# simplify23/MRN

Measured on AMD Instinct MI355X. Metric: text-line images/sec (fwd+bwd) at 32x256, TRBA+MRN 6 experts, higher is better.
Workload: dtype f32; 1 GPU; MRN loop B: TRBAx6 frozen experts fwd + DM-Router fwd/bwd + clip + Adam, 32x256x4 crops; per_gpu_batch=256, global_batch=256, parallelism=dp1

## Files before the change

mrn_amd/_lib.py:

```python
import ctypes
import os
import re

import torch

_HERE = os.path.dirname(os.path.abspath(__file__))
LIB_PATH = os.environ.get("MRN_LIB_PATH") or os.path.join(_HERE, "csrc", "libmrn_hip.so")
HEADER_PATH = os.path.join(os.path.dirname(_HERE), "include", "mrn_hip.h")
DECODE_HEADER_PATH = os.path.join(os.path.dirname(_HERE), "include", "mrn_decode.h")
ATTN_BEAM_HEADER_PATH = os.path.join(os.path.dirname(_HERE), "include", "mrn_attn_beam.h")
LEXICON_HEADER_PATH = os.path.join(os.path.dirname(_HERE), "include", "mrn_lexicon.h")
ATTN_LEXICON_HEADER_PATH = os.path.join(os.path.dirname(_HERE), "include", "mrn_attn_lexicon.h")

_CTYPES = {
    "int": ctypes.c_int,
    "int64_t": ctypes.c_int64,
    "float": ctypes.c_float,
    "void*": ctypes.c_void_p,
    "float*": ctypes.c_void_p,
    "const float*": ctypes.c_void_p,
    "const int64_t*": ctypes.c_void_p,
    "int64_t*": ctypes.c_void_p,
    "const int*": ctypes.c_void_p,
    "int*": ctypes.c_void_p,
    "const int32_t*": ctypes.c_void_p,
    "int32_t*": ctypes.c_void_p,
    "const void*": ctypes.c_void_p,
    "const void* const*": ctypes.c_void_p,
    "const char*": ctypes.c_char_p,
}


def parse_header(path=HEADER_PATH):
    text = open(path).read()
    text = re.sub(r"/\*.*?\*/", "", text, flags=re.S)
    text = re.sub(r"//[^\n]*", "", text)
    protos = {}
    for m in re.finditer(r"(?m)^\s*((?:const\s+)?\w+\s*\*?)\s*(mrn_\w+)\s*\(([^;{]*?)\)\s*;", text):
        ret = re.sub(r"\s+", " ", m.group(1)).strip().replace(" *", "*")
        name = m.group(2)
        args = m.group(3).strip()
        argtypes, argnames = [], []
        if args and args != "void":
            for a in args.split(","):
                a = re.sub(r"\s+", " ", a).strip()
                mm = re.match(r"(.*?)(\w+)$", a)
                ty = mm.group(1).strip().replace(" *", "*")
                argtypes.append(ty)
                argnames.append(mm.group(2))
        protos[name] = (ret, argtypes, argnames)
    return protos


class _Lib:
    def __init__(self):
        self._dll = None
        self._protos = None

    def load(self):
        if self._dll is not None:
            return self._dll
        if not os.path.exists(LIB_PATH):
            raise RuntimeError(
                f"{LIB_PATH} is missing: build it with `python -m mrn_amd.build` (there is no CPU fallback)")
        dll = ctypes.CDLL(LIB_PATH)
        self._protos = {**parse_header(), **parse_header(DECODE_HEADER_PATH), **parse_header(ATTN_BEAM_HEADER_PATH),
                        **parse_header(LEXICON_HEADER_PATH), **parse_header(ATTN_LEXICON_HEADER_PATH)}
        for name, (ret, argtypes, _) in self._protos.items():
            fn = getattr(dll, name)
            fn.restype = _CTYPES[ret]
            fn.argtypes = [_CTYPES[t] for t in argtypes]
        self._dll = dll
        return dll

    def call(self, name, *args):
        dll = self.load()
        fn = getattr(dll, name)
        rc = fn(*args)
        if fn.restype is ctypes.c_int and rc != 0:
            msg = dll.mrn_last_error().decode()
            raise RuntimeError(f"{name} failed (code {rc}): {msg}")
        return rc


LIB = _Lib()


def call(name, *args):
    return LIB.call(name, *args)
```

mrn_amd/csrc/group_ops.hip:

```cpp
#include "common.hpp"

namespace {

typedef _Float16 f16v8 __attribute__((ext_vector_type(8)));
typedef _Float16 f16v4 __attribute__((ext_vector_type(4)));

struct F8 {
  f32x4 a, b;
};

__device__ __forceinline__ F8 load8(const float* p) {
  F8 v;
  v.a = *reinterpret_cast<const f32x4*>(p);
  v.b = *reinterpret_cast<const f32x4*>(p + 4);
  return v;
}
__device__ __forceinline__ void store8(float* p, const F8& v) {
  *reinterpret_cast<f32x4*>(p) = v.a;
  *reinterpret_cast<f32x4*>(p + 4) = v.b;
}
__device__ __forceinline__ void store_hl(unsigned char* out, long row, int C, int c8, const F8& v) {
  f16v8 h, l;
#pragma unroll
  for (int e = 0; e < 4; ++e) {
    _Float16 hh, ll;
    split_f16_sat(v.a[e], hh, ll);
    h[e] = hh; l[e] = ll;
    split_f16_sat(v.b[e], hh, ll);
    h[4 + e] = hh; l[4 + e] = ll;
  }
  unsigned char* o = out + (row * (C >> 5) + (c8 >> 2)) * 128 + (c8 & 3) * 16;
  *reinterpret_cast<f16v8*>(o) = h;
  *reinterpret_cast<f16v8*>(o + 64) = l;
// ... 141 lines not shown
    }
    if (res || res_hl) {
      F8 r = res ? load8(res + i * 8) : load_hl(res_hl, row, C, c8);
      if constexpr (AFFINE) {
        const F8 rs = load8(res_scale + (long)g * C + c8 * 8), rt = load8(res_shift + (long)g * C + c8 * 8);
#pragma unroll
        for (int e = 0; e < 4; ++e) {
          r.a[e] = r.a[e] * rs.a[e] + rt.a[e];
          r.b[e] = r.b[e] * rs.b[e] + rt.b[e];
        }
      }
#pragma unroll
      for (int e = 0; e < 4; ++e) {
        v.a[e] += r.a[e];
        v.b[e] += r.b[e];
      }
    }
    if (relu == 1) {
#pragma unroll
      for (int e = 0; e < 4; ++e) {
        v.a[e] = relu_nan(v.a[e]);
        v.b[e] = relu_nan(v.b[e]);
      }
    } else if (relu == 2) {
#pragma unroll
      for (int e = 0; e < 4; ++e) {
        v.a[e] = 0.5f * v.a[e] * (1.f + erff(v.a[e] * 0.70710678118654752440f));
        v.b[e] = 0.5f * v.b[e] * (1.f + erff(v.b[e] * 0.70710678118654752440f));
      }
    }
    if (out) store8(out + i * 8, v);
    if (out_hl) store_hl(out_hl, row, C, c8, v);
  }
}

template <int R, bool AFFINE>
__global__ __launch_bounds__(256) void bn_apply_wino_grouped_kernel(const float* __restrict__ y, const float* __restrict__ res,
                                                                    const unsigned char* __restrict__ res_hl,
                                                                    const float* __restrict__ res_scale,
                                                                    const float* __restrict__ res_shift,
                                                                    const float* __restrict__ scale, const float* __restrict__ shift,
                                                                    float* __restrict__ out, unsigned char* __restrict__ out_hl,
                                                                    unsigned char* __restrict__ out_v, long imgrows_per_group, int W,
                                                                    int Wq, long n8, int C, int relu,
                                                                    const float* __restrict__ prescale, int dense) {
  constexpr int NC = R + 2;
  const float ps = prescale ? prescale[0] : 1.f;
  const int C8 = C >> 3, Cb = C >> 5;
  for (long i = blockIdx.x * 256L + threadIdx.x; i < n8; i += (long)gridDim.x * 256) {
    const int c8 = (int)(i % C8);
    const long t = i / C8;
    const int q = (int)(t % Wq);
    const long irow = t / Wq;
    const int g = (int)(irow / imgrows_per_group);
    F8 sc, sh;
    if (scale) {
      sc = load8(scale + (long)g * C + c8 * 8);
      sh = load8(shift + (long)g * C + c8 * 8);
    }
    F8 rs, rt;
    if constexpr (AFFINE) {
      rs = load8(res_scale + (long)g * C + c8 * 8);
      rt = load8(res_shift + (long)g * C + c8 * 8);
    }
    F8 d[NC];
#pragma unroll
    for (int j = 0; j < NC; ++j) {
      const int x = R * q - 1 + j;
      if ((unsigned)x < (unsigned)W) {
        const long row = irow * W + x;
        F8 v = load8(y + (row * C8 + c8) * 8);
        if (scale) {
#pragma unroll
          for (int e = 0; e < 4; ++e) {
            v.a[e] = v.a[e] * sc.a[e] + sh.a[e];
            v.b[e] = v.b[e] * sc.b[e] + sh.b[e];
          }
        }
        if (res || res_hl) {
          F8 r = res ? load8(res + (row * C8 + c8) * 8) : load_hl(res_hl, row, C, c8);
          if constexpr (AFFINE) {
#pragma unroll
            for (int e = 0; e < 4; ++e) {
              r.a[e] = r.a[e] * rs.a[e] + rt.a[e];
              r.b[e] = r.b[e] * rs.b[e] + rt.b[e];
            }
          }
#pragma unroll
          for (int e = 0; e < 4; ++e) {
            v.a[e] += r.a[e];
            v.b[e] += r.b[e];
          }
        }
        if (relu) {
#pragma unroll
          for (int e = 0; e < 4; ++e) {
            v.a[e] = relu_nan(v.a[e]);
            v.b[e] = relu_nan(v.b[e]);
          }
        }
        if (j >= 1 && j <= R) {
          if (out) store8(out + (row * C8 + c8) * 8, v);
          if (out_hl) store_hl(out_hl, row, C, c8, v);
        }
        d[j] = v;
      } else {
#pragma unroll
        for (int e = 0; e < 4; ++e) d[j].a[e] = d[j].b[e] = 0.f;
      }
    }
    F8 m[NC];
#pragma unroll
    for (int e = 0; e < 8; ++e) {
      auto D = [&](int j) { return e < 4 ? d[j].a[e] : d[j].b[e - 4]; };
      float r_[NC];
      if constexpr (R == 2) {
        r_[0] = D(0) - D(2);
        r_[1] = D(1) + D(2);
        r_[2] = D(2) - D(1);
        r_[3] = D(1) - D(3);
      } else {
        r_[0] = 4.f * D(0) - 5.f * D(2) + D(4);
        r_[1] = -4.f * (D(1) + D(2)) + D(3) + D(4);
        r_[2] = 4.f * (D(1) - D(2)) - D(3) + D(4);
        r_[3] = 2.f * (D(3) - D(1)) - D(2) + D(4);
        r_[4] = 2.f * (D(1) - D(3)) - D(2) + D(4);
        r_[5] = 4.f * D(1) - 5.f * D(3) + D(5);
      }
#pragma unroll
      for (int k = 0; k < NC; ++k) {
        if (e < 4) m[k].a[e] = r_[k] * ps;
        else m[k].b[e - 4] = r_[k] * ps;
      }
    }
#pragma unroll
    for (int k = 0; k < NC; ++k) {
      if (dense) store_d16(out_v, t * NC + k, C, c8, m[k], dense);
      else store_hl(out_v, t * NC + k, C, c8, m[k]);
    }
  }
}

__global__ __launch_bounds__(256) void maxpool_grouped_kernel(const float* __restrict__ x, const float* __restrict__ scale,
                                                              const float* __restrict__ shift, float* __restrict__ out,
                                                              unsigned char* __restrict__ out_hl, int relu, int B, long n8,
                                                              int H, int W, int C, int Ho, int Wo, int kh, int kw, int sh,
                                                              int sw, int ph, int pw) {
  const int C8 = C >> 3;
  for (long i = blockIdx.x * 256L + threadIdx.x; i < n8; i += (long)gridDim.x * 256) {
    const int c8 = (int)(i % C8);
    const long row = i / C8;
    long r = row;
    const int ox = (int)(r % Wo);
    r /= Wo;
    const int oy = (int)(r % Ho);
    const long b = r / Ho;
    const int g = (int)(b / B);
    F8 sc, sf;
    if (scale) {
      sc = load8(scale + (long)g * C + c8 * 8);
      sf = load8(shift + (long)g * C + c8 * 8);
    }
    F8 m;
#pragma unroll
    for (int e = 0; e < 4; ++e) m.a[e] = m.b[e] = -INFINITY;
    for (int ky = 0; ky < kh; ++ky) {
      const int iy = oy * sh - ph + ky;
      if ((unsigned)iy >= (unsigned)H) continue;
      for (int kx = 0; kx < kw; ++kx) {
        const int ix = ox * sw - pw + kx;
        if ((unsigned)ix >= (unsigned)W) continue;
// ... 30 lines not shown
                                                                   unsigned char* __restrict__ out_hl, unsigned char* __restrict__ out_v,
                                                                   int relu, int B, long n8, int H, int W, int C, int Ho, int Wo, int Wq,
                                                                   int kh, int kw, int sh, int sw, int ph, int pw, int dense) {
  constexpr int NC = R + 2;
  const int C8 = C >> 3;
  for (long i = blockIdx.x * 256L + threadIdx.x; i < n8; i += (long)gridDim.x * 256) {
    const int c8 = (int)(i % C8);
    const long t = i / C8;
    const int q = (int)(t % Wq);
    const long prow = t / Wq;
    const int oy = (int)(prow % Ho);
    const long b = prow / Ho;
    const int g = (int)(b / B);
    F8 sc, sf;
    if (scale) {
      sc = load8(scale + (long)g * C + c8 * 8);
      sf = load8(shift + (long)g * C + c8 * 8);
    }
    F8 d[NC];
#pragma unroll
    for (int j = 0; j < NC; ++j) {
      const int ox = R * q - 1 + j;
      if ((unsigned)ox < (unsigned)Wo) {
        F8 m;
#pragma unroll
        for (int e = 0; e < 4; ++e) m.a[e] = m.b[e] = -INFINITY;
        for (int ky = 0; ky < kh; ++ky) {
          const int iy = oy * sh - ph + ky;
          if ((unsigned)iy >= (unsigned)H) continue;
          for (int kx = 0; kx < kw; ++kx) {
            const int ix = ox * sw - pw + kx;
            if ((unsigned)ix >= (unsigned)W) continue;
            F8 v = load8(x + (((b * H + iy) * W + ix) * (long)C8 + c8) * 8);
            if (scale) {
#pragma unroll
              for (int e = 0; e < 4; ++e) {
                v.a[e] = v.a[e] * sc.a[e] + sf.a[e];
                v.b[e] = v.b[e] * sc.b[e] + sf.b[e];
              }
            }
#pragma unroll
            for (int e = 0; e < 4; ++e) {
              m.a[e] = max_nan(m.a[e], v.a[e]);
              m.b[e] = max_nan(m.b[e], v.b[e]);
            }
          }
        }
        if (relu) {
#pragma unroll
          for (int e = 0; e < 4; ++e) {
            m.a[e] = relu_nan(m.a[e]);
            m.b[e] = relu_nan(m.b[e]);
          }
        }
        if (j >= 1 && j <= R) {
          const long row = prow * Wo + ox;
          if (out) store8(out + (row * C8 + c8) * 8, m);
          if (out_hl) store_hl(out_hl, row, C, c8, m);
        }
        d[j] = m;
      } else {
#pragma unroll
        for (int e = 0; e < 4; ++e) d[j].a[e] = d[j].b[e] = 0.f;
      }
    }
    F8 m_[NC];
#pragma unroll
    for (int e = 0; e < 8; ++e) {
      auto D = [&](int j) { return e < 4 ? d[j].a[e] : d[j].b[e - 4]; };
      float r_[NC];
      if constexpr (R == 2) {
        r_[0] = D(0) - D(2);
        r_[1] = D(1) + D(2);
        r_[2] = D(2) - D(1);
        r_[3] = D(1) - D(3);
      } else {
        r_[0] = 4.f * D(0) - 5.f * D(2) + D(4);
        r_[1] = -4.f * (D(1) + D(2)) + D(3) + D(4);
        r_[2] = 4.f * (D(1) - D(2)) - D(3) + D(4);
        r_[3] = 2.f * (D(3) - D(1)) - D(2) + D(4);
        r_[4] = 2.f * (D(1) - D(3)) - D(2) + D(4);
        r_[5] = 4.f * D(1) - 5.f * D(3) + D(5);
      }
#pragma unroll
      for (int k = 0; k < NC; ++k) {
        if (e < 4) m_[k].a[e] = r_[k];
        else m_[k].b[e - 4] = r_[k];
      }
    }
#pragma unroll
    for (int k = 0; k < NC; ++k) {
      if (dense) store_d16(out_v, t * NC + k, C, c8, m_[k], dense);
      else store_hl(out_v, t * NC + k, C, c8, m_[k]);
    }
  }
}

template <int LPR>
__global__ __launch_bounds__(256) void add_layernorm_grouped_kernel(const float* __restrict__ x, const float* __restrict__ branch,
                                                                   const float* __restrict__ drop, long rows_per_drop,
                                                                   const float* __restrict__ gamma, const float* __restrict__ beta,
                                                                   long rows_per_group, float* __restrict__ sum_out,
                                                                   float* __restrict__ y_f32, unsigned char* __restrict__ y_hl,
                                                                   long rows, int C, float eps) {
  constexpr int RPW = 64 / LPR;
  constexpr int NV = 4;
  const int lane = threadIdx.x & 63, sub = lane % LPR;
  const long row = (blockIdx.x * 4L + (threadIdx.x >> 6)) * RPW + lane / LPR;
  if (row >= rows) return;
  const int C4 = C >> 2;
  const float* xr = x + row * C;
  f32x4 v[NV];
  float s = 0.f;
  const float ds = (branch && drop) ? drop[row / rows_per_drop] : 1.f;
#pragma unroll
  for (int i = 0; i < NV; ++i) {
    const int c4 = sub + i * LPR;
    v[i] = f32x4{0.f, 0.f, 0.f, 0.f};
    if (c4 < C4) {
      v[i] = reinterpret_cast<const f32x4*>(xr)[c4];
      if (branch) {
        const f32x4 b = reinterpret_cast<const f32x4*>(branch + row * C)[c4];
#pragma unroll
        for (int j = 0; j < 4; ++j) v[i][j] = fmaf(ds, b[j], v[i][j]);
      }
      if (sum_out) reinterpret_cast<f32x4*>(sum_out + row * C)[c4] = v[i];
// ... 177 lines not shown
                           const float* res_shift, const float* scale, const float* shift, float* out_f32, void* out_hl32, int G,
                           int64_t rows_per_group, int C, int relu, void* stream) {
  MRN_CHECK_ARG(y && (out_f32 || out_hl32) && C % 8 == 0 && (!(out_hl32 || residual_hl32) || C % 32 == 0) &&
                    (!scale == !shift) && !(residual && residual_hl32),
                "mrn_bn_apply_grouped_f32: bad operands (C=%d)", C);
  MRN_CHECK_ARG((!res_scale == !res_shift) && (!res_scale || (residual && !residual_hl32)),
                "mrn_bn_apply_grouped_res_affine_f32: the residual affine needs both vectors and the fp32 residual (C=%d)", C);
  const long n8 = (long)G * rows_per_group * (C / 8);
  if (n8 == 0) return MRN_OK;
  long grid = (n8 + 255) / 256;
  if (grid > 32768) grid = 32768;
  auto kernel = res_scale ? bn_apply_grouped_kernel<true> : bn_apply_grouped_kernel<false>;
  hipLaunchKernelGGL(kernel, dim3((unsigned)grid), dim3(256), 0, (hipStream_t)stream, y, residual,
                     (const unsigned char*)residual_hl32, res_scale, res_shift, scale, shift,
                     out_f32, (unsigned char*)out_hl32, (long)rows_per_group, n8, C, relu);
  MRN_LAUNCH_CHECK("bn_apply_grouped");
  return MRN_OK;
}

MRN_EXPORT int mrn_bn_apply_grouped_f32(const float* y, const float* residual, const void* residual_hl32, const float* scale,
                                        const float* shift, float* out_f32, void* out_hl32, int G, int64_t rows_per_group,
                                        int C, int relu, void* stream) {
  return bn_apply_launch(y, residual, residual_hl32, nullptr, nullptr, scale, shift, out_f32, out_hl32, G, rows_per_group, C, relu, stream);
}

MRN_EXPORT int mrn_bn_apply_grouped_res_affine_f32(const float* y, const float* residual, const void* residual_hl32,
                                                   const float* scale, const float* shift, float* out_f32, void* out_hl32, int G,
                                                   int64_t rows_per_group, int C, int relu, const float* res_scale,
                                                   const float* res_shift, void* stream) {
  return bn_apply_launch(y, residual, residual_hl32, res_scale, res_shift, scale, shift, out_f32, out_hl32, G, rows_per_group, C, relu,
                         stream);
}

static int bn_apply_wino_launch(const float* y, const float* residual, const void* residual_hl32, const float* res_scale,
                                const float* res_shift, const float* scale, const float* shift, float* out_f32, void* out_hl32,
                                void* out_wino, int G, int B, int H, int W, int C, int R, int relu, const float* prescale, int dense,
                                void* stream) {
  MRN_CHECK_ARG(y && out_wino && C % (dense ? 64 : 32) == 0 && (!scale == !shift) && !(residual && residual_hl32) && (R == 2 || R == 4) &&
                    out_f32 != y && (uintptr_t)out_wino % 128 == 0,
                "mrn_bn_apply_wino_grouped_f32: bad operands (C=%d R=%d)", C, R);
  MRN_CHECK_ARG((!res_scale == !res_shift) && (!res_scale || (residual && !residual_hl32)),
                "mrn_bn_apply_wino_grouped_res_affine_f32: the residual affine needs both vectors and the fp32 residual (C=%d)", C);
  const int Wq = (W + R - 1) / R;
  const long n8 = (long)G * B * H * Wq * (C / 8);
  if (n8 == 0) return MRN_OK;
  long grid = (n8 + 255) / 256;
  if (grid > 32768) grid = 32768;
  auto kernel = R == 4 ? (res_scale ? bn_apply_wino_grouped_kernel<4, true> : bn_apply_wino_grouped_kernel<4, false>)
                       : (res_scale ? bn_apply_wino_grouped_kernel<2, true> : bn_apply_wino_grouped_kernel<2, false>);
  hipLaunchKernelGGL(kernel, dim3((unsigned)grid), dim3(256), 0, (hipStream_t)stream, y, residual, (const unsigned char*)residual_hl32,
                     res_scale, res_shift, scale, shift, out_f32, (unsigned char*)out_hl32, (unsigned char*)out_wino, (long)B * H, W, Wq,
                     n8, C, relu, prescale, dense);
  MRN_LAUNCH_CHECK("bn_apply_wino_grouped");
  return MRN_OK;
}

MRN_EXPORT int mrn_bn_apply_wino_grouped_f32(const float* y, const float* residual, const void* residual_hl32, const float* scale,
                                             const float* shift, float* out_f32, void* out_hl32, void* out_wino, int G, int B, int H,
                                             int W, int C, int R, int relu, const float* prescale, void* stream) {
  return bn_apply_wino_launch(y, residual, residual_hl32, nullptr, nullptr, scale, shift, out_f32, out_hl32, out_wino, G, B, H, W, C, R, relu,
                              prescale, 0, stream);
}

MRN_EXPORT int mrn_bn_apply_wino_grouped_res_affine_f32(const float* y, const float* residual, const void* residual_hl32,
                                                        const float* scale, const float* shift, float* out_f32, void* out_hl32,
                                                        void* out_wino, int G, int B, int H, int W, int C, int R, int relu,
                                                        const float* prescale, const float* res_scale, const float* res_shift,
                                                        void* stream) {
  return bn_apply_wino_launch(y, residual, residual_hl32, res_scale, res_shift, scale, shift, out_f32, out_hl32, out_wino, G, B, H, W, C, R,
                              relu, prescale, 0, stream);
}

MRN_EXPORT int mrn_bn_apply_wino_grouped_d16_f32(const float* y, const float* residual, const void* residual_hl32, const float* scale,
                                                 const float* shift, float* out_f32, void* out_hl32, void* out_wino_d16, int G, int B, int H,
                                                 int W, int C, int relu, const float* prescale, int bf16, void* stream) {
  return bn_apply_wino_launch(y, residual, residual_hl32, nullptr, nullptr, scale, shift, out_f32, out_hl32, out_wino_d16, G, B, H, W, C, 4,
                              relu, prescale, bf16 ? 2 : 1, stream);
}

MRN_EXPORT int mrn_bn_apply_wino_grouped_d16_res_affine_f32(const float* y, const float* residual, const void* residual_hl32,
                                                            const float* scale, const float* shift, float* out_f32, void* out_hl32,
                                                            void* out_wino_d16, int G, int B, int H, int W, int C, int relu,
                                                            const float* prescale, int bf16, const float* res_scale,
                                                            const float* res_shift, void* stream) {
  return bn_apply_wino_launch(y, residual, residual_hl32, res_scale, res_shift, scale, shift, out_f32, out_hl32, out_wino_d16, G, B, H, W,
                              C, 4, relu, prescale, bf16 ? 2 : 1, stream);
}

MRN_EXPORT int mrn_maxpool_grouped_f32(const float* x, const float* scale, const float* shift, int relu, float* out_f32,
                                       void* out_hl32, int G, int B, int H, int W, int C, int kh, int kw, int sh, int sw, int ph,
                                       int pw, void* stream) {
  MRN_CHECK_ARG(x && (out_f32 || out_hl32) && C % 8 == 0 && (!out_hl32 || C % 32 == 0) && (!scale == !shift),
                "mrn_maxpool_grouped_f32: bad operands (C=%d)", C);
  const int Ho = (H + 2 * ph - kh) / sh + 1, Wo = (W + 2 * pw - kw) / sw + 1;
  MRN_CHECK_ARG(Ho > 0 && Wo > 0, "mrn_maxpool_grouped_f32: empty output");
  const long n8 = (long)G * B * Ho * Wo * (C / 8);
  if (n8 == 0) return MRN_OK;
  long grid = (n8 + 255) / 256;
  if (grid > 32768) grid = 32768;
  hipLaunchKernelGGL(maxpool_grouped_kernel, dim3((unsigned)grid), dim3(256), 0, (hipStream_t)stream, x, scale, shift, out_f32,
                     (unsigned char*)out_hl32, relu, B, n8, H, W, C, Ho, Wo, kh, kw, sh, sw, ph, pw);
  MRN_LAUNCH_CHECK("maxpool_grouped");
  return MRN_OK;
}

static int maxpool_wino_launch(const float* x, const float* scale, const float* shift, int relu, float* out_f32,
                               void* out_hl32, void* out_wino, int G, int B, int H, int W, int C, int kh, int kw, int sh,
                               int sw, int ph, int pw, int R, int dense, void* stream) {
  MRN_CHECK_ARG(x && out_wino && C % (dense ? 64 : 32) == 0 && (!scale == !shift) && (R == 2 || R == 4) && (uintptr_t)out_wino % 128 == 0,
                "mrn_maxpool_wino_grouped_f32: bad operands (C=%d R=%d)", C, R);
  const int Ho = (H + 2 * ph - kh) / sh + 1, Wo = (W + 2 * pw - kw) / sw + 1;
  MRN_CHECK_ARG(Ho > 0 && Wo > 0, "mrn_maxpool_wino_grouped_f32: empty output");
  const int Wq = (Wo + R - 1) / R;
  const long n8 = (long)G * B * Ho * Wq * (C / 8);
  if (n8 == 0) return MRN_OK;
  long grid = (n8 + 255) / 256;
  if (grid > 32768) grid = 32768;
  if (R == 4)
    hipLaunchKernelGGL(maxpool_wino_grouped_kernel<4>, dim3((unsigned)grid), dim3(256), 0, (hipStream_t)stream, x, scale, shift, out_f32,
                       (unsigned char*)out_hl32, (unsigned char*)out_wino, relu, B, n8, H, W, C, Ho, Wo, Wq, kh, kw, sh, sw, ph, pw, dense);
  else
    hipLaunchKernelGGL(maxpool_wino_grouped_kernel<2>, dim3((unsigned)grid), dim3(256), 0, (hipStream_t)stream, x, scale, shift, out_f32,
                       (unsigned char*)out_hl32, (unsigned char*)out_wino, relu, B, n8, H, W, C, Ho, Wo, Wq, kh, kw, sh, sw, ph, pw, dense);
  MRN_LAUNCH_CHECK("maxpool_wino_grouped");
  return MRN_OK;
}

MRN_EXPORT int mrn_maxpool_wino_grouped_f32(const float* x, const float* scale, const float* shift, int relu, float* out_f32,
                                            void* out_hl32, void* out_wino, int G, int B, int H, int W, int C, int kh, int kw, int sh,
                                            int sw, int ph, int pw, int R, void* stream) {
  return maxpool_wino_launch(x, scale, shift, relu, out_f32, out_hl32, out_wino, G, B, H, W, C, kh, kw, sh, sw, ph, pw, R, 0, stream);
}

MRN_EXPORT int mrn_maxpool_wino_grouped_d16_f32(const float* x, const float* scale, const float* shift, int relu, float* out_f32,
                                                void* out_hl32, void* out_wino_d16, int G, int B, int H, int W, int C, int kh, int kw, int sh,
                                                int sw, int ph, int pw, int bf16, void* stream) {
  return maxpool_wino_launch(x, scale, shift, relu, out_f32, out_hl32, out_wino_d16, G, B, H, W, C, kh, kw, sh, sw, ph, pw, 4, bf16 ? 2 : 1, stream);
}

MRN_EXPORT int mrn_add_layernorm_grouped_f32(const float* x, const float* branch, const float* drop, int64_t rows_per_drop,
                                             const float* gamma, const float* beta, int64_t rows_per_group, float* sum_out,
                                             float* y_f32, void* y_hl32, int64_t rows, int C, float eps, void* stream) {
  MRN_CHECK_ARG(x && (y_f32 || y_hl32 || sum_out) && C % 4 == 0 && C <= 1024 && (!y_hl32 || C % 32 == 0) && (!gamma == !beta) &&
                    rows_per_group >= 1 && (!drop || rows_per_drop >= 1),
                "mrn_add_layernorm_grouped_f32: bad operands (C=%d)", C);
  if (rows == 0) return MRN_OK;
  const hipStream_t st = (hipStream_t)stream;
  unsigned char* hl = (unsigned char*)y_hl32;
#define MRN_ALN_LAUNCH(LPR)                                                                                                   \
  hipLaunchKernelGGL(add_layernorm_grouped_kernel<LPR>, dim3((unsigned)((rows + 4 * (64 / LPR) - 1) / (4 * (64 / LPR)))),     \
                     dim3(256), 0, st, x, branch, drop, (long)rows_per_drop, gamma, beta, (long)rows_per_group, sum_out, y_f32,  \
// ... 9 lines not shown
```

mrn_amd/ops.py:

```python
import os
import sys
import weakref

import torch

from ._lib import call
from .modules.label_length import ctc_label_length_supported, ctc_uses_long_kernel, unsupported_label_length_message
from .modules.task_count import router_uses_wide_kernels, tasks_supported, unsupported_task_count_message

ACT_NONE, ACT_RELU, ACT_GELU = 0, 1, 2


class KernelTimer:

    def __init__(self, only=None):
        self.spans = []
        self.only = only

    def begin(self, site="other"):
        if self.only is not None and site not in self.only:
            return None
        e = torch.cuda.Event(enable_timing=True)
        e.record()
        return e
# ... 560 lines not shown
        else:
            call("mrn_pack_weight_wino_hl32", _p(w), out.data_ptr() + g * per, O, I, R, scale[g].data_ptr(), _stream())
    return out, scale


def bn_apply_wino_grouped(y, scale, shift, R, relu=True, residual=None, residual_hl=None, want_f32=False, want_hl=False, prescale=None,
                          dense=None, residual_affine=None):
    G, B, H, W, C = y.shape
    Wq = (W + R - 1) // R
    dense = wino_dense() if dense is None else dense
    eb = 2 if dense else 4
    out = torch.empty_like(y) if want_f32 else None
    out_hl = torch.empty(y.numel() * 4, device=y.device, dtype=torch.uint8) if want_hl else None
    v = torch.empty(G * B * H * Wq * (R + 2) * C * eb, device=y.device, dtype=torch.uint8)
    t0 = CONV_TIMER.begin("bnw") if CONV_TIMER is not None else None
    if residual_affine is not None:
        rs, rt = _residual_affine(residual_affine, residual, G, C)
        if dense:
            call("mrn_bn_apply_wino_grouped_d16_res_affine_f32", _p(y), _p(residual), _p(residual_hl), _p(scale), _p(shift), _p(out),
                 _p(out_hl), _p(v), G, B, H, W, C, int(bool(relu)), _p(prescale), int(REDUCED_BF16), _p(rs), _p(rt), _stream())
        else:
            call("mrn_bn_apply_wino_grouped_res_affine_f32", _p(y), _p(residual), _p(residual_hl), _p(scale), _p(shift), _p(out),
                 _p(out_hl), _p(v), G, B, H, W, C, R, int(bool(relu)), _p(prescale), _p(rs), _p(rt), _stream())
    elif dense:
        call("mrn_bn_apply_wino_grouped_d16_f32", _p(y), _p(residual), _p(residual_hl), _p(scale), _p(shift), _p(out), _p(out_hl), _p(v),
             G, B, H, W, C, int(bool(relu)), _p(prescale), int(REDUCED_BF16), _stream())
    else:
        call("mrn_bn_apply_wino_grouped_f32", _p(y), _p(residual), _p(residual_hl), _p(scale), _p(shift), _p(out), _p(out_hl), _p(v),
             G, B, H, W, C, R, int(bool(relu)), _p(prescale), _stream())
    if t0 is not None:
        n_io = 1 + int(residual is not None or residual_hl is not None) + int(want_f32) + int(want_hl)
        CONV_TIMER.end(t0, 0.0, "hbm/bn_apply_wino_grouped", 4.0 * y.numel() * n_io + float(eb) * G * B * H * Wq * (R + 2) * C)
    return out, out_hl, v


def wino_pool_supported(H, W, R, Cout):
    return PATCH_CONV and H % 2 == 0 and W % 2 == 0 and bool(call("mrn_conv2d_x3_wino_rows", H, R, Cout))


def conv2d_x3_wino(v_hl, G, shared_input, B, H, W, Cin, u_hl, u_scale, Cout, R, bias=None, act=ACT_NONE, want_stats=False, out=None,
                   x_scale=None, pool=False, gamma_ptrs=None, dense=None):
    dev = v_hl.device
    y = out if out is not None else torch.empty(G, B, H // 2 if pool else H, W // 2 if pool else W, Cout, device=dev, dtype=torch.float32)
    stats = None
    if want_stats:
        stats = torch.empty(call("mrn_conv2d_x3_wino_stats_floats", G, B, H, W, Cout, R), device=dev, dtype=torch.float32)
    Wq = (W + R - 1) // R
    dense = wino_dense() if dense is None else dense
    eb = 2 if dense else 4
    gstride = 0 if shared_input else B * H * Wq * (R + 2) * Cin * eb
    timed = CONV_TIMER is not None
    t0 = CONV_TIMER.begin("wino") if timed else None
    if dense:
        call("mrn_conv2d_x3_wino_d16", _p(v_hl), _p(u_hl), _p(bias), _p(y), _p(stats), _p(u_scale), _p(x_scale), G, gstride, B, H, W, Cin,
             Cout, act, int(bool(pool)), _p(gamma_ptrs), int(REDUCED_BF16), _stream())
    elif pool:
        call("mrn_conv2d_x3_wino_pool_hl32", _p(v_hl), _p(u_hl), _p(_zero_page(dev)), _p(bias), _p(y), _p(stats), _p(u_scale), _p(x_scale), G,
             gstride, B, H, W, Cin, Cout, R, act, _p(gamma_ptrs), _stream())
    else:
        call("mrn_conv2d_x3_wino_hl32", _p(v_hl), _p(u_hl), _p(_zero_page(dev)), _p(bias), _p(y), _p(stats), _p(u_scale), _p(x_scale), G,
             gstride, B, H, W, Cin, Cout, R, act, _stream())
    if WINO_CHECK and not pool and not dense and call("mrn_conv2d_x3_wino_rows", H, R, Cout):
        call("mrn_conv2d_x3_wino_select", 0)
        y2 = torch.empty_like(y)
        st2 = torch.empty(call("mrn_conv2d_x3_wino_stats_floats", G, B, H, W, Cout, R), device=dev, dtype=torch.float32) if want_stats else None
        call("mrn_conv2d_x3_wino_hl32", _p(v_hl), _p(u_hl), _p(_zero_page(dev)), _p(bias), _p(y2), _p(st2), _p(u_scale), _p(x_scale), G, gstride,
# ... 1854 lines not shown
```

Before: 3133 images/s.

## Walk Winograd tiles sequentially per thread to reuse overlapping BN and pool columns

The Winograd input producers (BN-apply and maxpool) now let each thread walk a run of consecutive tiles along a row. The overlapping halo columns carry over in registers instead of being reloaded and recomputed for every tile, and the next tile's loads are prefetched. Pooling windows also keep their overlapping columns between outputs. Split mode is chosen from C and Wq, or from an env var or select call. This cuts redundant global loads and recomputation, but lowers parallelism and raises register pressure.

Result: no change. 3140 images/s (median of 6 runs) (+0.2%).

```diff
diff --git a/include/mrn_wino_producer.h b/include/mrn_wino_producer.h
--- /dev/null
+++ b/include/mrn_wino_producer.h
@@ -0,0 +1,15 @@
+#ifndef MRN_WINO_PRODUCER_H
+#define MRN_WINO_PRODUCER_H
+#include <stdint.h>
+
+#ifdef __cplusplus
+extern "C" {
+#endif
+
+int mrn_wino_producer_select(int mode);
+int mrn_wino_producer_plan(int64_t rows, int Wq, int C, int split, int part, int64_t* plan);
+
+#ifdef __cplusplus
+}
+#endif
+#endif
diff --git a/mrn_amd/_lib.py b/mrn_amd/_lib.py
--- a/mrn_amd/_lib.py
+++ b/mrn_amd/_lib.py
@@ -11,6 +11,7 @@
 ATTN_BEAM_HEADER_PATH = os.path.join(os.path.dirname(_HERE), "include", "mrn_attn_beam.h")
 LEXICON_HEADER_PATH = os.path.join(os.path.dirname(_HERE), "include", "mrn_lexicon.h")
 ATTN_LEXICON_HEADER_PATH = os.path.join(os.path.dirname(_HERE), "include", "mrn_attn_lexicon.h")
+WINO_PRODUCER_HEADER_PATH = os.path.join(os.path.dirname(_HERE), "include", "mrn_wino_producer.h")
 
 _CTYPES = {
     "int": ctypes.c_int,
@@ -65,7 +66,8 @@
                 f"{LIB_PATH} is missing: build it with `python -m mrn_amd.build` (there is no CPU fallback)")
         dll = ctypes.CDLL(LIB_PATH)
         self._protos = {**parse_header(), **parse_header(DECODE_HEADER_PATH), **parse_header(ATTN_BEAM_HEADER_PATH),
-                        **parse_header(LEXICON_HEADER_PATH), **parse_header(ATTN_LEXICON_HEADER_PATH)}
+                        **parse_header(LEXICON_HEADER_PATH), **parse_header(ATTN_LEXICON_HEADER_PATH),
+                        **parse_header(WINO_PRODUCER_HEADER_PATH)}
         for name, (ret, argtypes, _) in self._protos.items():
             fn = getattr(dll, name)
             fn.restype = _CTYPES[ret]
diff --git a/mrn_amd/csrc/group_ops.hip b/mrn_amd/csrc/group_ops.hip
--- a/mrn_amd/csrc/group_ops.hip
+++ b/mrn_amd/csrc/group_ops.hip
@@ -1,4 +1,5 @@
 #include "common.hpp"
+#include <stdlib.h>
 
 namespace {
 
@@ -206,6 +207,151 @@
     if (out) store8(out + i * 8, v);
     if (out_hl) store_hl(out_hl, row, C, c8, v);
   }
+}
+
+
+struct WinoRaw {
+  F8 y, r;
+};
+
+__device__ __forceinline__ WinoRaw bnw_load(const float* __restrict__ y, const float* __restrict__ res,
+                                            const unsigned char* __restrict__ res_hl, long row, int C, int C8, int c8) {
+  WinoRaw w;
+  w.y = load8(y + (row * C8 + c8) * 8);
+  if (res) {
+    w.r = load8(res + (row * C8 + c8) * 8);
+  } else if (res_hl) {
+    const unsigned char* o = res_hl + (row * (C >> 5) + (c8 >> 2)) * 128 + (c8 & 3) * 16;
+    w.r.a = *reinterpret_cast<const f32x4*>(o);
+    w.r.b = *reinterpret_cast<const f32x4*>(o + 64);
+  }
+  return w;
+}
+
+template <bool AFFINE>
+__device__ __forceinline__ F8 bnw_eval(const WinoRaw& w, bool has_scale, bool res_f32, bool res_hl, const F8& sc, const F8& sh,
+                                       const F8& rs, const F8& rt, int relu) {
+  F8 v = w.y;
+  if (has_scale) {
+#pragma unroll
+    for (int e = 0; e < 4; ++e) {
+      v.a[e] = v.a[e] * sc.a[e] + sh.a[e];
+      v.b[e] = v.b[e] * sc.b[e] + sh.b[e];
+    }
+  }
+  if (res_f32 || res_hl) {
+    F8 r;
+    if (res_f32) {
+      r = w.r;
+    } else {
+      const f16v8 h = __builtin_bit_cast(f16v8, w.r.a), l = __builtin_bit_cast(f16v8, w.r.b);
+#pragma unroll
+      for (int e = 0; e < 4; ++e) {
+        r.a[e] = (float)h[e] + (float)l[e];
+        r.b[e] = (float)h[4 + e] + (float)l[4 + e];
+      }
+    }
+    if constexpr (AFFINE) {
+#pragma unroll
+      for (int e = 0; e < 4; ++e) {
+        r.a[e] = r.a[e] * rs.a[e] + rt.a[e];
+        r.b[e] = r.b[e] * rs.b[e] + rt.b[e];
+      }
+    }
+#pragma unroll
+    for (int e = 0; e < 4; ++e) {
+      v.a[e] += r.a[e];
+      v.b[e] += r.b[e];
+    }
+  }
+  if (relu) {
+#pragma unroll
+    for (int e = 0; e < 4; ++e) {
+      v.a[e] = relu_nan(v.a[e]);
+      v.b[e] = relu_nan(v.b[e]);
+    }
+  }
+  return v;
+}
+
+__device__ __forceinline__ F8 zero8() {
+  F8 z;
+#pragma unroll
+  for (int e = 0; e < 4; ++e) z.a[e] = z.b[e] = 0.f;
+  return z;
+}
+
+template <int R>
+__device__ __forceinline__ float wino_bt(int k, float d0, float d1, float d2, float d3, float d4, float d5) {
+  if constexpr (R == 2) {
+    switch (k) {
+      case 0: return d0 - d2;
+      case 1: return d1 + d2;
+      case 2: return d2 - d1;
+      default: return d1 - d3;
+    }
+  } else {
+    switch (k) {
+      case 0: return 4.f * d0 - 5.f * d2 + d4;
+      case 1: return -4.f * (d1 + d2) + d3 + d4;
+      case 2: return 4.f * (d1 - d2) - d3 + d4;
+      case 3: return 2.f * (d3 - d1) - d2 + d4;
+      case 4: return 2.f * (d1 - d3) - d2 + d4;
+      default: return 4.f * d1 - 5.f * d3 + d5;
+    }
+  }
+}
+
+template <int R, bool PRESCALE, bool SEQ>
+__device__ __forceinline__ void wino_bt_store(const F8 (&d)[R + 2], float ps, unsigned char* __restrict__ out_v, long t, int C, int c8,
+                                              int dense) {
+  constexpr int NC = R + 2;
+#pragma unroll
+  for (int k = 0; k < NC; ++k) {
+    F8 m;
+#pragma unroll
+    for (int e = 0; e < 8; ++e) {
+      auto D = [&](int j) { return e < 4 ? d[j < NC ? j : NC - 1].a[e] : d[j < NC ? j : NC - 1].b[e - 4]; };
+      const float r_ = wino_bt<R>(k, D(0), D(1), D(2), D(3), D(4), D(5));
+      const float val = PRESCALE ? r_ * ps : r_;
+      if (e < 4) m.a[e] = val;
+      else m.b[e - 4] = val;
+    }
+    if (dense) store_d16(out_v, t * NC + k, C, c8, m, dense);
+    else store_hl(out_v, t * NC + k, C, c8, m);
+    if (SEQ) __builtin_amdgcn_sched_barrier(0);
+  }
+}
+
+__device__ __forceinline__ F8 pool_affine(F8 v, const F8& sc, const F8& sf) {
+#pragma unroll
+  for (int e = 0; e < 4; ++e) {
+    v.a[e] = v.a[e] * sc.a[e] + sf.a[e];
+    v.b[e] = v.b[e] * sc.b[e] + sf.b[e];
+  }
+  return v;
+}
+__device__ __forceinline__ F8 pool_max(F8 m, const F8& v) {
+#pragma unroll
+  for (int e = 0; e < 4; ++e) {
+    m.a[e] = max_nan(m.a[e], v.a[e]);
+    m.b[e] = max_nan(m.b[e], v.b[e]);
+  }
+  return m;
+}
+__device__ __forceinline__ F8 relu8(F8 m) {
+#pragma unroll
+  for (int e = 0; e < 4; ++e) {
+    m.a[e] = relu_nan(m.a[e]);
+    m.b[e] = relu_nan(m.b[e]);
+  }
+  return m;
+}
+
+__host__ __device__ inline void wino_walk_run(int Wq, int split, int part, int& q0, int& q1) {
+  const int base = Wq / split, rem = Wq % split;
+  q0 = part * base + (part < rem ? part : rem);
+  q1 = q0 + base + (part < rem ? 1 : 0);
 }
 
 template <int R, bool AFFINE>
@@ -243,74 +389,102 @@
       const int x = R * q - 1 + j;
       if ((unsigned)x < (unsigned)W) {
         const long row = irow * W + x;
-        F8 v = load8(y + (row * C8 + c8) * 8);
-        if (scale) {
-#pragma unroll
-          for (int e = 0; e < 4; ++e) {
-            v.a[e] = v.a[e] * sc.a[e] + sh.a[e];
-            v.b[e] = v.b[e] * sc.b[e] + sh.b[e];
-          }
-        }
-        if (res || res_hl) {
-          F8 r = res ? load8(res + (row * C8 + c8) * 8) : load_hl(res_hl, row, C, c8);
-          if constexpr (AFFINE) {
-#pragma unroll
-            for (int e = 0; e < 4; ++e) {
-              r.a[e] = r.a[e] * rs.a[e] + rt.a[e];
-              r.b[e] = r.b[e] * rs.b[e] + rt.b[e];
-            }
-          }
-#pragma unroll
-          for (int e = 0; e < 4; ++e) {
-            v.a[e] += r.a[e];
-            v.b[e] += r.b[e];
-          }
-        }
-        if (relu) {
-#pragma unroll
-          for (int e = 0; e < 4; ++e) {
-            v.a[e] = relu_nan(v.a[e]);
-            v.b[e] = relu_nan(v.b[e]);
-          }
-        }
+        const F8 v = bnw_eval<AFFINE>(bnw_load(y, res, res_hl, row, C, C8, c8), scale != nullptr, res != nullptr, res_hl != nullptr, sc, sh,
+                                      rs, rt, relu);
         if (j >= 1 && j <= R) {
           if (out) store8(out + (row * C8 + c8) * 8, v);
           if (out_hl) store_hl(out_hl, row, C, c8, v);
         }
         d[j] = v;
       } else {
-#pragma unroll
-        for (int e = 0; e < 4; ++e) d[j].a[e] = d[j].b[e] = 0.f;
-      }
-    }
-    F8 m[NC];
-#pragma unroll
-    for (int e = 0; e < 8; ++e) {
-      auto D = [&](int j) { return e < 4 ? d[j].a[e] : d[j].b[e - 4]; };
-      float r_[NC];
-      if constexpr (R == 2) {
-        r_[0] = D(0) - D(2);
-        r_[1] = D(1) + D(2);
-        r_[2] = D(2) - D(1);
-        r_[3] = D(1) - D(3);
-      } else {
-        r_[0] = 4.f * D(0) - 5.f * D(2) + D(4);
-        r_[1] = -4.f * (D(1) + D(2)) + D(3) + D(4);
-        r_[2] = 4.f * (D(1) - D(2)) - D(3) + D(4);
-        r_[3] = 2.f * (D(3) - D(1)) - D(2) + D(4);
-        r_[4] = 2.f * (D(1) - D(3)) - D(2) + D(4);
-        r_[5] = 4.f * D(1) - 5.f * D(3) + D(5);
-      }
-#pragma unroll
-      for (int k = 0; k < NC; ++k) {
-        if (e < 4) m[k].a[e] = r_[k] * ps;
-        else m[k].b[e - 4] = r_[k] * ps;
-      }
-    }
-#pragma unroll
-    for (int k = 0; k < NC; ++k) {
-      if (dense) store_d16(out_v, t * NC + k, C, c8, m[k], dense);
-      else store_hl(out_v, t * NC + k, C, c8, m[k]);
+        d[j] = zero8();
+      }
+    }
+    wino_bt_store<R, true, false>(d, ps, out_v, t, C, c8, dense);
+  }
+}
+
+template <int R, bool AFFINE, int SPLIT, int RES>
+__global__ __launch_bounds__(256) void bn_apply_wino_grouped_kernel(const float* __restrict__ y, const float* __restrict__ res_,
+                                                                    const unsigned char* __restrict__ res_hl_,
+                                                                    const float* __restrict__ res_scale,
+                                                                    const float* __restrict__ res_shift,
+                                                                    const float* __restrict__ scale, const float* __restrict__ shift,
+                                                                    float* __restrict__ out, unsigned char* __restrict__ out_hl,
+                                                                    unsigned char* __restrict__ out_v, long imgrows_per_group, int W,
+                                                                    int Wq, long n8, int C, int relu,
+                                                                    const float* __restrict__ prescale, int dense) {
+  constexpr int NC = R + 2;
+  const float ps = prescale ? prescale[0] : 1.f;
+  const int C8 = C >> 3;
+  const float* __restrict__ res = RES == 1 ? res_ : nullptr;
+  const unsigned char* __restrict__ res_hl = RES == 2 ? res_hl_ : nullptr;
+  const bool has_scale = scale != nullptr, res_f32 = res != nullptr, res_h = res_hl != nullptr;
+  for (long i = xcd_remap((int)blockIdx.x, (int)gridDim.x) * 256L + threadIdx.x; i < n8; i += (long)gridDim.x * 256) {
+    const int c8 = (int)(i % C8);
+    const long u = i / C8;
+    const int part = (int)(u % SPLIT);
+    const long irow = u / SPLIT;
+    int q0, q1;
+    wino_walk_run(Wq, SPLIT, part, q0, q1);
+    if (q0 >= q1) continue;
+    const int g = (int)(irow / imgrows_per_group);
+    F8 sc, sh;
+    if (scale) {
+      sc = load8(scale + (long)g * C + c8 * 8);
+      sh = load8(shift + (long)g * C + c8 * 8);
+    }
+    F8 rs, rt;
+    if constexpr (AFFINE) {
+      rs = load8(res_scale + (long)g * C + c8 * 8);
+      rt = load8(res_shift + (long)g * C + c8 * 8);
+    }
+    const long row0 = irow * W;
+    const int xend = R * q1 < W ? R * q1 : W;
+    F8 d[NC];
+    {
+      const int x = R * q0;
+      d[0] = x > 0 ? bnw_eval<AFFINE>(bnw_load(y, res, res_hl, row0 + x - 1, C, C8, c8), has_scale, res_f32, res_h, sc, sh, rs, rt, relu)
+                   : zero8();
+      d[1] = bnw_eval<AFFINE>(bnw_load(y, res, res_hl, row0 + x, C, C8, c8), has_scale, res_f32, res_h, sc, sh, rs, rt, relu);
+      if (out) store8(out + ((row0 + x) * C8 + c8) * 8, d[1]);
+      if (out_hl) store_hl(out_hl, row0 + x, C, c8, d[1]);
+    }
+    WinoRaw cur[R];
+#pragma unroll
+    for (int j = 0; j < R; ++j) {
+      const int x = R * q0 + 1 + j;
+      cur[j] = bnw_load(y, res, res_hl, row0 + (x < W ? x : W - 1), C, C8, c8);
+    }
+    for (int q = q0; q < q1; ++q) {
+#pragma unroll
+      for (int j = 0; j < R; ++j) {
+        const int x = R * q + 1 + j;
+        const F8 v = bnw_eval<AFFINE>(cur[j], has_scale, res_f32, res_h, sc, sh, rs, rt, relu);
+#pragma unroll
+        for (int e = 0; e < 4; ++e) {
+          d[2 + j].a[e] = x < W ? v.a[e] : 0.f;
+          d[2 + j].b[e] = x < W ? v.b[e] : 0.f;
+        }
+      }
+      if (q + 1 < q1 && R * (q + 1) + 1 < W) {
+#pragma unroll
+        for (int j = 0; j < R; ++j) {
+          const int x = R * (q + 1) + 1 + j;
+          cur[j] = bnw_load(y, res, res_hl, row0 + (x < W ? x : W - 1), C, C8, c8);
+        }
+      }
+#pragma unroll
+      for (int j = 0; j < R; ++j) {
+        const int x = R * q + 1 + j;
+        if (x < xend) {
+          if (out) store8(out + ((row0 + x) * C8 + c8) * 8, d[2 + j]);
+          if (out_hl) store_hl(out_hl, row0 + x, C, c8, d[2 + j]);
+        }
+      }
+      wino_bt_store<R, true, true>(d, ps, out_v, irow * Wq + q, C, c8, dense);
+      d[0] = d[R];
+      d[1] = d[R + 1];
     }
   }
 }
@@ -407,27 +581,11 @@
             const int ix = ox * sw - pw + kx;
             if ((unsigned)ix >= (unsigned)W) continue;
             F8 v = load8(x + (((b * H + iy) * W + ix) * (long)C8 + c8) * 8);
-            if (scale) {
-#pragma unroll
-              for (int e = 0; e < 4; ++e) {
-                v.a[e] = v.a[e] * sc.a[e] + sf.a[e];
-                v.b[e] = v.b[e] * sc.b[e] + sf.b[e];
-              }
-            }
-#pragma unroll
-            for (int e = 0; e < 4; ++e) {
-              m.a[e] = max_nan(m.a[e], v.a[e]);
-              m.b[e] = max_nan(m.b[e], v.b[e]);
-            }
+            if (scale) v = pool_affine(v, sc, sf);
+            m = pool_max(m, v);
           }
         }
-        if (relu) {
-#pragma unroll
-          for (int e = 0; e < 4; ++e) {
-            m.a[e] = relu_nan(m.a[e]);
-            m.b[e] = relu_nan(m.b[e]);
-          }
-        }
+        if (relu) m = relu8(m);
         if (j >= 1 && j <= R) {
           const long row = prow * Wo + ox;
           if (out) store8(out + (row * C8 + c8) * 8, m);
@@ -435,38 +593,125 @@
         }
         d[j] = m;
       } else {
-#pragma unroll
-        for (int e = 0; e < 4; ++e) d[j].a[e] = d[j].b[e] = 0.f;
-      }
-    }
-    F8 m_[NC];
-#pragma unroll
-    for (int e = 0; e < 8; ++e) {
-      auto D = [&](int j) { return e < 4 ? d[j].a[e] : d[j].b[e - 4]; };
-      float r_[NC];
-      if constexpr (R == 2) {
-        r_[0] = D(0) - D(2);
-        r_[1] = D(1) + D(2);
-        r_[2] = D(2) - D(1);
-        r_[3] = D(1) - D(3);
+        d[j] = zero8();
+      }
+    }
+    wino_bt_store<R, false, false>(d, 1.f, out_v, t, C, c8, dense);
+  }
+}
+
+template <int KH, int KW, int SW, bool FRESH>
+__device__ __forceinline__ F8 pool_walk_column(const float* __restrict__ x, const long (&rowoff)[KH], const bool (&vy)[KH], int ox, int pw,
+                                               int W, int C8, int c8, bool has_scale, const F8& sc, const F8& sf, int relu,
+                                               F8 (&keep)[KH][KW > SW ? KW - SW : 1]) {
+  constexpr int KOV = KW > SW ? KW - SW : 0;
+  F8 win[KH][KW];
+#pragma unroll
+  for (int ky = 0; ky < KH; ++ky) {
+#pragma unroll
+    for (int kx = 0; kx < KW; ++kx) {
+      const int ix = ox * SW - pw + kx;
+      if (!FRESH && kx < KOV) {
+        win[ky][kx] = keep[ky][kx];
       } else {
-        r_[0] = 4.f * D(0) - 5.f * D(2) + D(4);
-        r_[1] = -4.f * (D(1) + D(2)) + D(3) + D(4);
-        r_[2] = 4.f * (D(1) - D(2)) - D(3) + D(4);
-        r_[3] = 2.f * (D(3) - D(1)) - D(2) + D(4);
-        r_[4] = 2.f * (D(1) - D(3)) - D(2) + D(4);
-        r_[5] = 4.f * D(1) - 5.f * D(3) + D(5);
-      }
-#pragma unroll
-      for (int k = 0; k < NC; ++k) {
-        if (e < 4) m_[k].a[e] = r_[k];
-        else m_[k].b[e - 4] = r_[k];
-      }
-    }
-#pragma unroll
-    for (int k = 0; k < NC; ++k) {
-      if (dense) store_d16(out_v, t * NC + k, C, c8, m_[k], dense);
-      else store_hl(out_v, t * NC + k, C, c8, m_[k]);
+        const int ixc = ix < 0 ? 0 : (ix < W ? ix : W - 1);
+        win[ky][kx] = load8(x + ((rowoff[ky] + ixc) * (long)C8 + c8) * 8);
+        if (has_scale) win[ky][kx] = pool_affine(win[ky][kx], sc, sf);
+      }
+    }
+  }
+  F8 m;
+#pragma unroll
+  for (int e = 0; e < 4; ++e) m.a[e] = m.b[e] = -INFINITY;
+#pragma unroll
+  for (int ky = 0; ky < KH; ++ky) {
+#pragma unroll
+    for (int kx = 0; kx < KW; ++kx) {
+      const int ix = ox * SW - pw + kx;
+      const F8 mm = pool_max(m, win[ky][kx]);
+      const bool valid = vy[ky] && (unsigned)ix < (unsigned)W;
+#pragma unroll
+      for (int e = 0; e < 4; ++e) {
+        m.a[e] = valid ? mm.a[e] : m.a[e];
+        m.b[e] = valid ? mm.b[e] : m.b[e];
+      }
+    }
+  }
+  if (relu) m = relu8(m);
+#pragma unroll
+  for (int ky = 0; ky < KH; ++ky) {
+#pragma unroll
+    for (int k = 0; k < KOV; ++k) keep[ky][k] = win[ky][k + SW];
+  }
+  return m;
+}
+
+template <int R, int SPLIT, int KH, int KW, int SW>
+__global__ __launch_bounds__(256) void maxpool_wino_grouped_kernel(const float* __restrict__ x, const float* __restrict__ scale,
+                                                                   const float* __restrict__ shift, float* __restrict__ out,
+                                                                   unsigned char* __restrict__ out_hl, unsigned char* __restrict__ out_v,
+                                                                   int relu, int B, long n8, int H, int W, int C, int Ho, int Wo, int Wq,
+                                                                   int sh, int ph, int pw, int dense) {
+  constexpr int NC = R + 2;
+  const int C8 = C >> 3;
+  const bool has_scale = scale != nullptr;
+  for (long i = xcd_remap((int)blockIdx.x, (int)gridDim.x) * 256L + threadIdx.x; i < n8; i += (long)gridDim.x * 256) {
+    const int c8 = (int)(i % C8);
+    const long u = i / C8;
+    const int part = (int)(u % SPLIT);
+    const long prow = u / SPLIT;
+    int q0, q1;
+    wino_walk_run(Wq, SPLIT, part, q0, q1);
+    if (q0 >= q1) continue;
+    const int oy = (int)(prow % Ho);
+    const long b = prow / Ho;
+    const int g = (int)(b / B);
+    F8 sc, sf;
+    if (scale) {
+      sc = load8(scale + (long)g * C + c8 * 8);
+      sf = load8(shift + (long)g * C + c8 * 8);
+    }
+    long rowoff[KH];
+    bool vy[KH];
+#pragma unroll
+    for (int ky = 0; ky < KH; ++ky) {
+      const int iy = oy * sh - ph + ky;
+      vy[ky] = (unsigned)iy < (unsigned)H;
+      rowoff[ky] = (b * H + (vy[ky] ? iy : 0)) * W;
+    }
+    const long orow0 = prow * Wo;
+    const int xend = R * q1 < Wo ? R * q1 : Wo;
+    F8 keep[KH][KW > SW ? KW - SW : 1];
+    F8 d[NC];
+    {
+      const int ox = R * q0;
+      if (ox > 0) {
+        d[0] = pool_walk_column<KH, KW, SW, true>(x, rowoff, vy, ox - 1, pw, W, C8, c8, has_scale, sc, sf, relu, keep);
+        d[1] = pool_walk_column<KH, KW, SW, false>(x, rowoff, vy, ox, pw, W, C8, c8, has_scale, sc, sf, relu, keep);
+      } else {
+        d[0] = zero8();
+        d[1] = pool_walk_column<KH, KW, SW, true>(x, rowoff, vy, ox, pw, W, C8, c8, has_scale, sc, sf, relu, keep);
+      }
+      if (out) store8(out + ((orow0 + ox) * C8 + c8) * 8, d[1]);
+      if (out_hl) store_hl(out_hl, orow0 + ox, C, c8, d[1]);
+    }
+    for (int q = q0; q < q1; ++q) {
+#pragma unroll
+      for (int j = 0; j < R; ++j) {
+        const int ox = R * q + 1 + j;
+        d[2 + j] = ox < Wo ? pool_walk_column<KH, KW, SW, false>(x, rowoff, vy, ox, pw, W, C8, c8, has_scale, sc, sf, relu, keep) : zero8();
+      }
+#pragma unroll
+      for (int j = 0; j < R; ++j) {
+        const int ox = R * q + 1 + j;
+        if (ox < xend) {
+          if (out) store8(out + ((orow0 + ox) * C8 + c8) * 8, d[2 + j]);
+          if (out_hl) store_hl(out_hl, orow0 + ox, C, c8, d[2 + j]);
+        }
+      }
+      wino_bt_store<R, false, true>(d, 1.f, out_v, prow * Wq + q, C, c8, dense);
+      d[0] = d[R];
+      d[1] = d[R + 1];
     }
   }
 }
@@ -710,6 +955,43 @@
                          stream);
 }
 
+static int g_walk_mode = -1;
+
+MRN_EXPORT int mrn_wino_producer_select(int mode) {
+  MRN_CHECK_ARG(mode == -1 || mode == 0 || mode == 1 || mode == 4, "mrn_wino_producer_select: mode %d (-1, 0, 1 or 4)", mode);
+  g_walk_mode = mode;
+  return MRN_OK;
+}
+
+static int wino_walk_split(int Wq, int C) {
+  static const int env = getenv("MRN_WINO_WALK") ? atoi(getenv("MRN_WINO_WALK")) : -1;
+  const int mode = g_walk_mode >= 0 ? g_walk_mode : env;
+  if (mode == 0 || mode == 1 || mode == 4) return mode;
+  if (C >= 512) return 0;
+  return C <= 128 && Wq >= 4 ? 4 : 1;
+}
+
+static void wino_walk_plan(long rows, int Wq, int C, int split, long& n8, long& grid) {
+  n8 = rows * (split ? split : Wq) * (C / 8);
+  grid = (n8 + 255) / 256;
+  if (grid > 32768) grid = 32768;
+}
+
+MRN_EXPORT int mrn_wino_producer_plan(int64_t rows, int Wq, int C, int split, int part, int64_t* plan) {
+  MRN_CHECK_ARG(plan && rows >= 0 && Wq >= 1 && C >= 8 && C % 8 == 0 && (split == 0 || split == 1 || split == 4) && part >= 0 &&
+                    part < (split ? split : 1),
+                "mrn_wino_producer_plan: bad arguments (Wq=%d C=%d split=%d part=%d)", Wq, C, split, part);
+  long n8, grid;
+  wino_walk_plan((long)rows, Wq, C, split, n8, grid);
+  int q0 = 0, q1 = Wq;
+  if (split) wino_walk_run(Wq, split, part, q0, q1);
+  plan[0] = n8;
+  plan[1] = grid;
+  plan[2] = q0;
+  plan[3] = q1;
+  return MRN_OK;
+}
+
 static int bn_apply_wino_launch(const float* y, const float* residual, const void* residual_hl32, const float* res_scale,
                                 const float* res_shift, const float* scale, const float* shift, float* out_f32, void* out_hl32,
                                 void* out_wino, int G, int B, int H, int W, int C, int R, int relu, const float* prescale, int dense,
@@ -720,12 +1002,23 @@
   MRN_CHECK_ARG((!res_scale == !res_shift) && (!res_scale || (residual && !residual_hl32)),
                 "mrn_bn_apply_wino_grouped_res_affine_f32: the residual affine needs both vectors and the fp32 residual (C=%d)", C);
   const int Wq = (W + R - 1) / R;
-  const long n8 = (long)G * B * H * Wq * (C / 8);
+  const int split = wino_walk_split(Wq, C);
+  long n8, grid;
+  wino_walk_plan((long)G * B * H, Wq, C, split, n8, grid);
   if (n8 == 0) return MRN_OK;
-  long grid = (n8 + 255) / 256;
-  if (grid > 32768) grid = 32768;
   auto kernel = R == 4 ? (res_scale ? bn_apply_wino_grouped_kernel<4, true> : bn_apply_wino_grouped_kernel<4, false>)
                        : (res_scale ? bn_apply_wino_grouped_kernel<2, true> : bn_apply_wino_grouped_kernel<2, false>);
+#define MRN_BNW_WALK(S_)                                                                                                  \
+  do {                                                                                                                    \
+    if (res_scale) kernel = R == 4 ? bn_apply_wino_grouped_kernel<4, true, S_, 1> : bn_apply_wino_grouped_kernel<2, true, S_, 1>; \
+    else if (residual) kernel = R == 4 ? bn_apply_wino_grouped_kernel<4, false, S_, 1> : bn_apply_wino_grouped_kernel<2, false, S_, 1>; \
+    else if (residual_hl32)                                                                                               \
+      kernel = R == 4 ? bn_apply_wino_grouped_kernel<4, false, S_, 2> : bn_apply_wino_grouped_kernel<2, false, S_, 2>;    \
+    else kernel = R == 4 ? bn_apply_wino_grouped_kernel<4, false, S_, 0> : bn_apply_wino_grouped_kernel<2, false, S_, 0>; \
+  } while (0)
+  if (split == 1) MRN_BNW_WALK(1);
+  else if (split == 4) MRN_BNW_WALK(4);
+#undef MRN_BNW_WALK
   hipLaunchKernelGGL(kernel, dim3((unsigned)grid), dim3(256), 0, (hipStream_t)stream, y, residual, (const unsigned char*)residual_hl32,
                      res_scale, res_shift, scale, shift, out_f32, (unsigned char*)out_hl32, (unsigned char*)out_wino, (long)B * H, W, Wq,
                      n8, C, relu, prescale, dense);
@@ -790,11 +1083,28 @@
   const int Ho = (H + 2 * ph - kh) / sh + 1, Wo = (W + 2 * pw - kw) / sw + 1;
   MRN_CHECK_ARG(Ho > 0 && Wo > 0, "mrn_maxpool_wino_grouped_f32: empty output");
   const int Wq = (Wo + R - 1) / R;
-  const long n8 = (long)G * B * Ho * Wq * (C / 8);
+  const bool walkable = kh == 2 && ((kw == 2 && (sw == 2 || sw == 1)) || (kw == 1 && sw == 1));
+  const int split = walkable ? wino_walk_split(Wq, C) : 0;
+  long n8, grid;
+  wino_walk_plan((long)G * B * Ho, Wq, C, split, n8, grid);
   if (n8 == 0) return MRN_OK;
-  long grid = (n8 + 255) / 256;
-  if (grid > 32768) grid = 32768;
-  if (R == 4)
+  if (split) {
+#define MRN_POOL_WALK(R_, S_, KW_, SW_)                                                                                                  \
+  hipLaunchKernelGGL((maxpool_wino_grouped_kernel<R_, S_, 2, KW_, SW_>), dim3((unsigned)grid), dim3(256), 0, (hipStream_t)stream, x, scale, \
+                     shift, out_f32, (unsigned char*)out_hl32, (unsigned char*)out_wino, relu, B, n8, H, W, C, Ho, Wo, Wq, sh, ph, pw, dense)
+#define MRN_POOL_WALK_RS(KW_, SW_)                                     \
+  do {                                                                 \
+    if (R == 4 && split == 1) MRN_POOL_WALK(4, 1, KW_, SW_);           \
+    else if (R == 4) MRN_POOL_WALK(4, 4, KW_, SW_);                    \
+    else if (split == 1) MRN_POOL_WALK(2, 1, KW_, SW_);                \
+    else MRN_POOL_WALK(2, 4, KW_, SW_);                                \
+  } while (0)
+    if (kw == 2 && sw == 2) MRN_POOL_WALK_RS(2, 2);
+    else if (kw == 2) MRN_POOL_WALK_RS(2, 1);
+    else MRN_POOL_WALK_RS(1, 1);
+#undef MRN_POOL_WALK_RS
+#undef MRN_POOL_WALK
+  } else if (R == 4)
     hipLaunchKernelGGL(maxpool_wino_grouped_kernel<4>, dim3((unsigned)grid), dim3(256), 0, (hipStream_t)stream, x, scale, shift, out_f32,
                        (unsigned char*)out_hl32, (unsigned char*)out_wino, relu, B, n8, H, W, C, Ho, Wo, Wq, kh, kw, sh, sw, ph, pw, dense);
   else
diff --git a/mrn_amd/ops.py b/mrn_amd/ops.py
--- a/mrn_amd/ops.py
+++ b/mrn_amd/ops.py
@@ -616,6 +616,10 @@
         n_io = 1 + int(residual is not None or residual_hl is not None) + int(want_f32) + int(want_hl)
         CONV_TIMER.end(t0, 0.0, "hbm/bn_apply_wino_grouped", 4.0 * y.numel() * n_io + float(eb) * G * B * H * Wq * (R + 2) * C)
     return out, out_hl, v
+
+
+def wino_producer_select(mode):
+    call("mrn_wino_producer_select", int(mode))
 
 
 def wino_pool_supported(H, W, R, Cout):
```
